# mkln/spamtree

Hardware: AMD Instinct MI355X
Metric: Gibbs iterations/sec + achieved HBM GB/s, n=1e6 grid, 1/2/4/8 MI355X (higher is better)
Workload: dtype f64

## Files before the change

### profiles/micro/stamps.py

```python
import ctypes as C
import os
import sys

import numpy as np

ROOT = os.path.dirname(os.path.dirname(os.path.dirname(os.path.abspath(__file__))))
sys.path.insert(0, ROOT)
from spamtree_amd import _lib

_lib.LIB_PATH = os.path.join(ROOT, "profiles", "micro", "libspamtree_hip_stamps.so")
from spamtree_amd.model import SpamTreeMV
from spamtree_amd.synthetic import make_workload

NAMES = {0: "topology+coords", 1: "covariance", 2: "private ancestor step", 3: "panel barrier wait", 4: "panel compute (MFMA)",
         5: "DMA wait + pad", 6: "DMA issue", 7: "cholesky", 8: "N = -Ri T + store", 9: "final barrier", 10: "hv", 11: "R / leaf outputs",
         12: "Ri out + e2", 13: "scalars"}

side = int(sys.argv[1]) if len(sys.argv) > 1 else 1000
q = int(sys.argv[2]) if len(sys.argv) > 2 else 1
cell = int(sys.argv[3]) if len(sys.argv) > 3 else 25
missing = tuple(float(x) for x in sys.argv[4].split(",")) if len(sys.argv) > 4 else None
wl = make_workload(side, q=q, cell_size=cell, missing=missing, device=0)
hm = SpamTreeMV(wl["y"], wl["X"], wl["Z"], wl["coords"], wl["mv_id"], wl["blocking"], wl["gix_block"], wl["res_is_ref"],
                wl["parents"], wl["children"], False, wl["block_names"], wl["block_groups"], wl["indexing"],
                np.zeros(wl["n"]), np.zeros(wl["p"]), wl["theta"], 10.0, device=0)
lib = hm.lib
lib.st_debug_stamps.argtypes = [C.POINTER(C.c_ulonglong), C.c_int]
lib.st_debug_stamp_level.argtypes = [C.c_int]
hm.get_loglik_comps_w(0)
nlev = len(np.unique(np.asarray(wl["block_groups"])))
for lev in range(max(0, nlev - 4), nlev):
    lib.st_debug_stamp_level(lev)
    buf = (C.c_ulonglong * 16)()
    lib.st_debug_stamps(buf, 1)
    for _ in range(3):
        hm.get_loglik_comps_w(1)
    lib.st_debug_stamps(buf, 0)
    v = np.array(list(buf), dtype=np.float64)
    tot = v.sum()
    if tot == 0:
        continue
    print(f"level {lev}: total ticks {tot:.3e}")
    for i in np.argsort(-v):
        if v[i] > 0:
            print(f"   {NAMES.get(int(i), str(i)):28s} {100 * v[i] / tot:5.1f} %")
hm.close()
```

### spamtree_amd/csrc/factor_quad.hpp

```cpp
#pragma once

struct Quad {
  int g0, nu;
  int Jc, Pc;
};

struct QuadArgs {
  const Blk *blks;
  const int *anc_idx;
  const Grp *grps;
  const Quad *quads;
  int nquad;
  const double *cx, *cy;
  const int *mv;
  const double *w;
  double *panels;
  double *logdet_c, *loglik_c;
  int *errflag;
  const long long *gdesc;
  int gd_stride;
  int ldS;
  int wave_chol;
  int predict;
  const double *z;
  double *w_out;
  int mode;
  double *vscr;
  int vtiles;
};

enum { QM_FULL = 0, QM_VONLY = 1, QM_TFROMV = 2 };
__host__ __device__ constexpr int quad_vtiles(int nkx) { return 2 + 2 * ((4 * nkx + 31) / 32); }

#define RFL(x) __builtin_amdgcn_readfirstlane(x)

constexpr int QUAD_LEAF_KH = 5;
__host__ __device__ constexpr int quad_lds_stride(int nkx) {
  int s = 4 * nkx + 24 > 186 ? 4 * nkx + 24 : 186;
  while ((s & 1) || ((s >> 1) & 1) == 0) ++s;
  return s;
}

#ifdef ST_DEFS_FACTOR_QUAD
__device__ __forceinline__ void dma_row(const double *src, double *dst, int Kb, int lane, bool two) {
  if (2 * lane < Kb) __builtin_amdgcn_global_load_lds((q_glb_void *)(src + 2 * lane), (q_lds_void *)dst, 16, 0, 0);
  if (two) {
    if (128 + 2 * lane < Kb) __builtin_amdgcn_global_load_lds((q_glb_void *)(src + 128 + 2 * lane), (q_lds_void *)(dst + 128), 16, 0, 0);
  }
}

template <int NU, int NKX, int NKT, bool ISREF, bool WCH = true>
__global__ __launch_bounds__(128 * NU, 2) void k_factor_quad(QuadArgs A, CovPar cp) {
  constexpr int NTQ = 128 * NU, NW = 2 * NU;
  static_assert(NU >= 2, "s_g overlays two rows of s_e2");
  constexpr int PMAX = 4 * NKX, KH = ISREF ? (NKX + 3) / 4 : QUAD_LEAF_KH, NPASS = (NKX + KH - 1) / KH;
  static_assert(NKT * 16 >= PMAX, "T tiles must cover the chain");
  extern __shared__ double lds[];
  __shared__ int s_am[MAXJ], s_ao[MAXJ + 1];
  __shared__ long long s_arow[MAXJ], s_apan[MAXJ];
  __shared__ int s_uM[NU], s_uP[NU], s_ublk0[NU], s_unblk[NU], s_uref[NU], s_uJ[NU], s_pm[NU], s_fail[NU], s_level;
  __shared__ long long s_urow0[NU], s_prow[NU], s_ppan[NU];
  constexpr int NB = ISREF ? 1 : 32, NUL = ISREF ? 1 : NU;
  __shared__ long long s_bpan[NU][NB], s_brow[NU][NB];
  __shared__ int s_bld[NU][NB];
  __shared__ double s_colx[NU][32], s_coly[NU][32], s_colw[NU][32], s_hv[NU][32];
  __shared__ double s_px[NUL][32], s_py[NUL][32], s_pw[NUL][32];
  __shared__ double s_e2[NU][32], s_lg[NU][32];
  __shared__ int s_colmv[NU][32], s_colblk[NUL][32], s_pmv[NUL][32];
  __shared__ int s_nit;
  __shared__ double s_sx[PMAX], s_sy[PMAX], s_wpa[PMAX];
  __shared__ int s_smv[PMAX];
  __shared__ double s_exp2[64];
  __shared__ double s_cvr[QMAX * QMAX], s_cva[QMAX * QMAX], s_cva2[QMAX * QMAX], s_cvp[QMAX];
  __shared__ int s_rlen[PMAX];
  __shared__ long long s_rsrc[PMAX];
  double (*s_g)[32] = s_e2;
  double (*s_gp)[32] = s_hv;

  auto body = [&](auto qmc) __attribute__((always_inline)) {
  constexpr int QM = decltype(qmc)::value;
  const int tid = threadIdx.x, lane = tid & 63, l15 = lane & 15, l4 = lane >> 4, ttid = tid & 127;
  const int wid = RFL(tid >> 6), u = wid >> 1, jt = (wid & 1) ^ ((wid >> 2) & 1);
  constexpr int ldS = quad_lds_stride(NKX);
  double *arena = lds;
  double *zrow = arena + (size_t)NU * 16 * ldS;
  double *xch = zrow + ldS;

  STAMP_DECL
  int qidx = blockIdx.x;
  {
    const int per = A.nquad >> 3;
    if (qidx < per * 8) qidx = (qidx & 7) * per + (qidx >> 3);
  }
  const Quad Q = A.quads[qidx];
  const int Jc = Q.Jc, Pc = Q.Pc, nu = Q.nu;

  long long *gdl = (long long *)arena;
  const int gds = A.gd_stride;
  for (int e = tid; e < nu * gds; e += NTQ) {
    const int uu = e / gds, i = e - uu * gds;
    gdl[e] = A.gdesc[(size_t)(Q.g0 + uu) * gds + i];
  }
  for (int k = tid; k < ldS; k += NTQ) zrow[k] = 0.0;
  if (tid < 64) s_exp2[tid] = EXP2_64[tid];
  if (cp.q > 1 && tid >= 64 && tid < 64 + QMAX * QMAX) {
    const int e = tid - 64;
    s_cvr[e] = cp.rate[e]; s_cva[e] = cp.amp[e]; s_cva2[e] = cp.amp2[e];
    if (e < QMAX) s_cvp[e] = cp.phi[e];
  }
  __syncthreads();
  if (tid < NU) {
    int M = 0, P = 0, blk0 = 0, nblk = 0, isref = 0, J = 0, pm = 0;
    long long row0 = 0, prow = 0, ppan = 0;
    if (tid < nu) {
      const long long *g = gdl + (size_t)tid * gds;
      row0 = g[0];
      M = (int)(g[2] & 0xffffffffLL); P = (int)(g[2] >> 32);
      J = (int)(g[3] & 0xffffffffLL); nblk = (int)(g[3] >> 32);
      isref = (int)(g[4] & 0xffffffffLL);
      blk0 = (int)(g[6] & 0xffffffffLL);
      if (tid == 0) s_level = (int)(g[4] >> 32);
      if (J > Jc) {
        const long long *a = g + 8 + 4 * Jc;
        pm = (int)(a[0] & 0xffffffffLL); prow = a[1]; ppan = a[2];
      }
    }
    s_uM[tid] = M; s_uP[tid] = P; s_ublk0[tid] = blk0; s_unblk[tid] = nblk; s_uref[tid] = isref; s_uJ[tid] = J;
    s_pm[tid] = pm; s_urow0[tid] = row0; s_prow[tid] = prow; s_ppan[tid] = ppan; s_fail[tid] = 0;
  }
  if (tid >= 64 && tid < 64 + Jc) {
    const int t = tid - 64;
    const long long *a = gdl + 8 + 4 * t;
    s_am[t] = (int)(a[0] & 0xffffffffLL); s_ao[t] = (int)(a[0] >> 32); s_arow[t] = a[1]; s_apan[t] = a[2];
  }
  if (tid == 32) {
    s_ao[Jc] = Pc;
    s_nit = (Pc + 31) >> 5;
  }
  for (int e = tid; e < NU * NB; e += NTQ) {
    const int uu = e / NB, b = e - uu * NB;
    if (uu < nu) {
      const long long *g = gdl + (size_t)uu * gds;
      const int J = (int)(g[3] & 0xffffffffLL), nblk = (int)(g[3] >> 32);
      if (b < nblk) {
        const long long *q = g + 8 + 4 * J + 3 * b;
        s_bpan[uu][b] = q[0]; s_brow[uu][b] = q[1]; s_bld[uu][b] = (int)q[2];
      }
    }
  }
  __syncthreads();
  const int Mu = RFL(s_uM[u]), Pu = RFL(s_uP[u]), pmu = RFL(s_pm[u]);
  constexpr bool isref = ISREF;
  const bool wact = jt * 16 < Mu;
  const bool two = Mu > 16;
  int Mmax = 0, pmmax = 0;
#pragma unroll
  for (int i = 0; i < NU; ++i) { Mmax = max(Mmax, s_uM[i]); pmmax = max(pmmax, s_pm[i]); }
  Mmax = RFL(Mmax); pmmax = RFL(pmmax);
  constexpr bool anyref = ISREF;

  for (int k = tid; k < Pc; k += NTQ) {
    int t = 0;
#pragma unroll
    for (int j = 1; j < 8; ++j) t += (j < Jc && k >= s_ao[j]) ? 1 : 0;
    for (int j = 8; j < Jc; ++j) t += (k >= s_ao[j]) ? 1 : 0;
    const long long r = s_arow[t] + (k - s_ao[t]);
    s_sx[k] = A.cx[r]; s_sy[k] = A.cy[r]; s_smv[k] = A.mv[r]; s_wpa[k] = A.w[r];
    const int len = s_ao[t + 1];
    s_rlen[k] = len; s_rsrc[k] = s_apan[t] + (long long)(k - s_ao[t]) * len;
  }
  for (int e = tid; e < NU * 32; e += NTQ) {
    const int uu = e >> 5, i = e & 31;
    double x = 0.0, y = 0.0, ww = 0.0; int v = 0;
    if constexpr (!ISREF) {
      if (i < s_pm[uu]) { const long long r = s_prow[uu] + i; x = A.cx[r]; y = A.cy[r]; ww = A.w[r]; v = A.mv[r]; }
      s_px[uu][i] = x; s_py[uu][i] = y; s_pw[uu][i] = ww; s_pmv[uu][i] = v;
      x = 0.0; y = 0.0; ww = 0.0; v = 0;
    }
    int bi = 0;
    if (i < s_uM[uu]) {
      const long long r = s_urow0[uu] + i;
      x = A.cx[r]; y = A.cy[r]; ww = A.w[r]; v = A.mv[r];
      if constexpr (!ISREF) { while (bi + 1 < s_unblk[uu] && r >= s_brow[uu][bi + 1]) ++bi; }
    }
    s_colx[uu][i] = x; s_coly[uu][i] = y; s_colw[uu][i] = ww; s_colmv[uu][i] = v;
    if constexpr (!ISREF) s_colblk[uu][i] = bi;
  }
  __syncthreads();

  STAMP(0);
  const int p_sr0 = pmu > 16 ? (pmu + 1) >> 1 : pmu;
  const int p_Kb = Pc + pmu;
  constexpr int RP = 32 / NW;
  const int nit = RFL(s_nit);
  int rlen_cur[RP], rlen_nx[RP];
#pragma unroll
  for (int rr = 0; rr < RP; ++rr) { rlen_cur[rr] = 0; rlen_nx[rr] = 0; }
  auto issue = [&](int i, double *buf) {
    const int c0 = 32 * (nit - 1 - i), sr = min(32, Pc - c0);
    int lv[RP];
    long long sv[RP];
#pragma unroll
    for (int rr = 0; rr < RP; ++rr) {
// ... 63 lines not shown
            double v = s_cva[ij] * cov_exp_tab(-s_cvr[ij] * hd, s_exp2);
            v = fma(s_cva2[ij], cov_exp_tab(-s_cvp[av] * hd, s_exp2), v);
            kb[i * 64] = (cok && k < Pu) ? v : 0.0;
          }
        }
#pragma unroll
        for (int i = 0; i < KH; ++i)
          if (st0 + i < NKX) kx[st0 + i] = kb[i * 64];
      } else {
#pragma unroll
        for (int i = 0; i < KH; ++i)
          if (st0 + i < NKX) kx[st0 + i] = 0.0;
      }
    }
  }
  STAMP(1);
  d4 tacc[NKT];
#pragma unroll
  for (int n = 0; n < NKT; ++n) tacc[n] = (d4){0.0, 0.0, 0.0, 0.0};
  d4 rown = (d4){0.0, 0.0, 0.0, 0.0}, rcross = rown;
  double dacc = 0.0;
  double hacc = 0.0;
  const size_t vq0 = ((size_t)qidx * A.vtiles * NW + wid) * 256;
  auto vstore = [&](int t, const d4 &p) __attribute__((always_inline)) {
    double *d = A.vscr + (vq0 + (size_t)t * (NW * 256)) + lane;
    __builtin_nontemporal_store(p[0], d); __builtin_nontemporal_store(p[1], d + 64);
    __builtin_nontemporal_store(p[2], d + 128); __builtin_nontemporal_store(p[3], d + 192);
  };
  auto vload = [&](int t) __attribute__((always_inline)) {
    const double *d = A.vscr + (vq0 + (size_t)t * (NW * 256)) + lane;
// ... 98 lines not shown
          double gv = 0.0;
          if (row < sr) gv = grow(buf + (size_t)row * ldS, p_Kb, Pc, s_pw[u], lane & 7, std::integral_constant<int, 8>());
          if ((lane & 7) == 0) s_gp[u][r0 + row] = gv;
        }
        lds_barrier();
        if (sp == 1 && pf) issue(0, arena + (size_t)48 * ldS);
        if (sr > 0) {
          tile(buf, (sr + 3) >> 2, min(p_Kb, Pc + r0 + sr), 0, sr, &s_gp[u][r0], kget(16 + 4 * sp), sp);
        }
        lds_barrier();
      }
    }
  }

  STAMP(2);
  {
    if constexpr (!ISREF) { if (nit > 0 && !pf) issue(0, arena); }
    int cur = pf ? 1 : 0;
    if (QM == QM_TFROMV && wact && nit > 0) { kset(0, vload(2)); if (Pc - 32 * (nit - 1) > 16) kset(4, vload(3)); }
    for (int i = 0; i < nit; ++i) {
      const int c0 = 32 * (nit - 1 - i), sr = min(32, Pc - c0);
      const int kb_v = s_rlen[c0 + sr - 1], kba_v = s_rlen[c0 + min(sr, 16) - 1];
      const int Kb = RFL(kb_v), KbA0 = RFL(kba_v);
      double *buf = arena + (size_t)((pf && i == 0) ? 48 : cur * 32) * ldS;
#pragma unroll
      for (int rr = 0; rr < RP; ++rr) rlen_cur[rr] = rlen_nx[rr];
      asm volatile("s_waitcnt vmcnt(0)" ::: "memory");
#pragma unroll
      for (int rr = 0; rr < RP; ++rr) {
        const int row = wid + NW * rr;
// ... 15 lines not shown
        if (lane % NS == 0) s_g[cur][row] = gv;
      }
      STAMP(5);
      lds_barrier();
      STAMP(3);
      if (i + 1 < nit) issue(i + 1, arena + (size_t)(cur ^ 1) * 32 * ldS);
      if (QM == QM_TFROMV && wact && i + 1 < nit) { kset(8, vload(2 * i + 4)); if (Pc - 32 * (nit - 2 - i) > 16) kset(12, vload(2 * i + 5)); }
      STAMP(6);
      compute(buf, sr, min(Kb, c0 + 32), min(KbA0, c0 + 16), ISREF ? nullptr : s_g[cur], kget(0), kget(4), 2 + 2 * i);
      if (QM == QM_TFROMV) { kset(0, kget(8)); kset(4, kget(12)); }
      STAMP(4);
      cur ^= 1;
    }
  }
  lds_barrier();

  double h0 = 0.0, h1 = 0.0, h2 = 0.0, h3 = 0.0;
  if (QM == QM_FULL && (ISREF || A.predict)) {
#pragma unroll
    for (int n = 0; n < NKT; ++n) {
      const int k = n * 16 + l15;
      double wv = k < Pc ? s_wpa[k] : 0.0;
      if constexpr (!ISREF) { if (k >= Pc && k < Pu) wv = s_pw[u][k - Pc]; }
      h0 += tacc[n][0] * wv; h1 += tacc[n][1] * wv; h2 += tacc[n][2] * wv; h3 += tacc[n][3] * wv;
    }
#pragma unroll
    for (int o = 1; o < 16; o <<= 1) {
      h0 += __shfl_xor(h0, o, 64); h1 += __shfl_xor(h1, o, 64); h2 += __shfl_xor(h2, o, 64); h3 += __shfl_xor(h3, o, 64);
    }
    if (l15 == 0) {
// ... 299 lines not shown
```

### spamtree_amd/csrc/spamtree_hip.hip

```cpp

#include <unordered_map>

#include "tree_layout.hpp"
#include "misc_kernels.hpp"
#include "predict_points.hpp"
#include "predict_joint.hpp"
#include "simulate_kernels.hpp"

static thread_local std::string g_create_error;
struct st_handle_s;
static void points_free(st_handle_s *h);

template <typename T>
struct DevBuf {
  T *p = nullptr;
  size_t n = 0;
  DevBuf() = default;
  DevBuf(const DevBuf &) = delete;
  DevBuf &operator=(const DevBuf &) = delete;
  DevBuf(DevBuf &&o) noexcept : p(o.p), n(o.n) { o.p = nullptr; o.n = 0; }
  DevBuf &operator=(DevBuf &&o) noexcept { if (this != &o) { free(); p = o.p; n = o.n; o.p = nullptr; o.n = 0; } return *this; }
  ~DevBuf() { free(); }
  hipError_t alloc(size_t count) {
    n = count;
// ... 30 lines not shown
  "k_factor_quad<4, 50, 13, true, true>", "k_factor_quad<4, 50, 13, true, false>", "k_factor_quad<4, 50, 13, false, true>",
  "k_factor_mfma", "k_factor_lchain<96>", "k_factor_lchain<136>", "k_factor_ref_finish", "k_lchain_scalars", "k_factor_wide<WG_JT>",
  "k_factor_bigmfma<3, 5, 34>", "k_factor_bigmfma<4, 5, 34>", "k_factor_bigmfma<5, 3, 24>",
  "k_gram", "k_gram_direct", "k_gram_big",
  "k_sample_mfma", "k_sample_leaf_seg<4>", "k_sample_leaf_seg<6>", "k_sample_leaf", "k_sample_wave", "k_sample_lean<true>",
  "k_sample_lean<false>", "k_sample<true, false>", "k_sample_leaf_wide", "k_sample<true, true>", "k_sample<false>",
};

struct st_handle_s : TreeLayout {
  std::string err;
  int device = 0;
  hipStream_t stream = nullptr;
  int quirks = 1;
  long long n_obs = 0;
  DevBuf<Grp> d_grps;
  DevBuf<Quad> d_quads;
  DevBuf<WideGrp> d_wgrps;
  DevBuf<LcSlab> d_lcslabs;
  DevBuf<long long> d_rfvoff, d_gdesc;
  DevBuf<double> d_vscr;
  DevBuf<double> d_lcrow;
  DevBuf<double> d_s0;
  DevBuf<long long> d_s0off;
  bool c_pending = false;
  int c_rc = 0; double c_ll = 0.0;
  DevBuf<int> d_ownobs, d_owngrp, d_ownslow;
  DevBuf<unsigned char> d_rowmask, d_blkmask;
  DevBuf<double> d_comm;
  DevBuf<double> d_gather;
  DevBuf<int> d_gidx;
  DevBuf<double> d_gerr;
// ... 244 lines not shown
  CCHK(h->d_mv.upload(mv)); CCHK(h->d_obs.upload(obs)); CCHK(h->d_partner.upload(partner));
  CCHK(h->d_dev2model.upload(h->dev2model));
  return ST_OK;
}

static int create_layout_buffers(st_handle_s *h) {
  {
    std::vector<Blk> db = h->blks;
    if (h->limited) for (Blk &B : db) B.acc_len = 0;
    CCHK(h->d_blks.upload(db));
    if (h->limited) CCHK(upload_or_dummy(h->d_twin, h->twin_list));
  }
  CCHK(upload_or_dummy(h->d_anc, h->anc_idx)); CCHK(upload_or_dummy(h->d_dch, h->dch_idx));
  CCHK(h->d_lvl.upload(h->lvl_list));
  CCHK(upload_or_dummy(h->d_grps, h->grps)); CCHK(h->d_gdesc.upload(h->gdesc));
  CCHK(upload_or_dummy(h->d_quads, h->quads)); CCHK(upload_or_dummy(h->d_wgrps, h->wgrps));
  if (!h->lcslabs.empty()) { CCHK(h->d_lcslabs.upload(h->lcslabs)); CCHK(h->d_lcrow.alloc((size_t)2 * h->n_all)); }
  if (!h->rfvoff.empty()) { CCHK(h->d_rfvoff.upload(h->rfvoff)); CCHK(h->d_vscr.alloc(h->vscr_need + (size_t)2 * RF_BUFD)); }
  CCHK(h->d_s0off.upload(h->s0off));
  CCHK(h->d_s0.alloc(std::max(h->s0_total, (size_t)1)));
  CCHK(upload_or_dummy(h->d_pred, h->pred_list));
  CCHK(h->d_allobs.upload(h->all_obs_list));
  CCHK(upload_or_dummy(h->d_ownobs, h->own_obs_list));
  CCHK(upload_or_dummy(h->d_owngrp, h->own_grp_list)); CCHK(upload_or_dummy(h->d_ownslow, h->own_obs_slow));
  CCHK(h->d_rowmask.upload(h->rowmask)); CCHK(h->d_blkmask.upload(h->blkmask));
  CCHK(h->d_comm.alloc((size_t)2 * h->n_blocks + 64));
  CCHK(h->d_gidx.upload(h->gidx));
  CCHK(h->d_gather.alloc(h->gidx.size()));
  CCHK(h->d_gerr.alloc(64));
  CCHK(upload_or_dummy(h->d_toplist, h->top_list));
  CCHK(h->d_err2.alloc(2));
// ... 162 lines not shown
  if (h->top_pending) { HCHK(h, hipSetDevice(h->device)); HCHK(h, hipStreamWaitEvent(h->stream, h->ev_top, 0)); }
  return ST_OK;
}
static int complete_leaf(st_handle h, int slot) {
  const int phys = h->slot_map[slot];
  if (!h->leaf_pending[phys]) return ST_OK;
  HCHK(h, hipSetDevice(h->device));
  const CovPar &cp = h->leaf_cp[phys];
  ProfScope phase(h, 0, -2, 0);
  for (int g = 0; g < h->n_actual_groups; ++g) {
    const LevelInfo &L = h->levels[g];
    if (L.vl_off < 0) continue;
    QuadArgs F;
    std::memset(&F, 0, sizeof(F));
    F.blks = h->d_blks.p; F.anc_idx = h->d_anc.p; F.grps = h->d_grps.p + L.grp_first;
    F.quads = h->d_quads.p + L.quad_first + L.qown_lo; F.nquad = L.qown_n;
    F.cx = h->d_cx.p; F.cy = h->d_cy.p; F.mv = h->d_mv.p; F.w = h->d_w.p; F.panels = h->d_panels[phys].p;
    F.errflag = h->d_err.p; F.ldS = L.q_ldS;
    F.gdesc = h->d_gdesc.p + (size_t)L.grp_first * h->gd_stride; F.gd_stride = h->gd_stride;
    F.wave_chol = L.maxM <= 27 ? 1 : 0;
    F.mode = QM_TFROMV; F.vscr = h->d_vleaf.p + L.vl_off; F.vtiles = quad_vtiles(L.q_nkx);
    ProfScope ps(h, 0, g, 0);
#define QT(NU_, NKX_, NKT_) hipLaunchKernelGGL((k_factor_quad<NU_, NKX_, NKT_, false, true>), dim3(L.qown_n), dim3(128 * NU_), L.lds_quad, h->stream, F, cp)
    if (L.q_nkx == 32) QT(4, 32, 8); else if (L.q_nkx == 38) QT(4, 38, 10); else if (L.q_nkx == 44) QT(4, 44, 11); else QT(4, 50, 13);
#undef QT
    HCHK(h, hipGetLastError());
  }
  h->leaf_pending[phys] = false;
  return ST_OK;
}
extern "C" int st_swap(st_handle h) {
  if (!h) return ST_ERR_USAGE;
  if (h->top_pending) {
    h->err = "st_swap between st_factor_begin and the st_factor / st_factor_local that picks its result up";
// ... 116 lines not shown
  for (int g = g_lo; g < g_hi; ++g) {
    const LevelInfo &L = h->levels[g];
    if ((L.fast ? L.gown_n : L.own_n) == 0) continue;
    FactorArgs A;
    std::memset(&A, 0, sizeof(A));
    A.blks = h->d_blks.p; A.anc_idx = h->d_anc.p; A.list = h->d_lvl.p + L.first + L.own_lo; A.nlist = L.own_n;
    A.cx = h->d_cx.p; A.cy = h->d_cy.p; A.mv = h->d_mv.p; A.w_in = h->d_w.p; A.w_out = nullptr; A.z = nullptr;
    A.panels = h->d_panels[phys].p; A.logdet_c = h->d_logdet[phys].p; A.loglik_c = h->d_loglik[phys].p;
    A.errflag = errflag; A.maxP = L.maxP; A.maxM = L.maxM; A.maxMa = L.maxMa; A.SR = L.big_factor ? 4 : 8;
    {
      ProfScope ps(h, 0, g, 1, st);
      if (L.fast && h->sw.factor_gen == 3 && L.q_nkx > 0) {
        QuadArgs F;
        std::memset(&F, 0, sizeof(F));
        F.blks = h->d_blks.p; F.anc_idx = h->d_anc.p; F.grps = h->d_grps.p + L.grp_first;
        F.quads = h->d_quads.p + L.quad_first + L.qown_lo; F.nquad = L.qown_n;
        F.cx = h->d_cx.p; F.cy = h->d_cy.p; F.mv = h->d_mv.p; F.w = h->d_w.p; F.panels = h->d_panels[phys].p;
        F.logdet_c = h->d_logdet[phys].p; F.loglik_c = h->d_loglik[phys].p; F.errflag = errflag; F.ldS = L.q_ldS;
        F.gdesc = h->d_gdesc.p + (size_t)L.grp_first * h->gd_stride; F.gd_stride = h->gd_stride;
        F.wave_chol = L.maxM <= 27 ? 1 : 0;
#define QLAUNCH(NU_, NKX_, NKT_, R_)     \
  do {                                                                                                                         \
    if (L.isref && F.wave_chol) { route(g, R_); hipLaunchKernelGGL((k_factor_quad<NU_, NKX_, NKT_, true, true>), dim3(L.qown_n), dim3(128 * NU_), L.lds_quad, st, F, cp); } \
    else if (L.isref) { route(g, R_ + 1); hipLaunchKernelGGL((k_factor_quad<NU_, NKX_, NKT_, true, false>), dim3(L.qown_n), dim3(128 * NU_), L.lds_quad, st, F, cp); } \
    else {                                                                                                                     \
      if (vonly && L.vl_off >= 0) { F.mode = QM_VONLY; F.vscr = h->d_vleaf.p + L.vl_off; F.vtiles = quad_vtiles(NKX_); *deferred = true; } \
      route(g, R_ + 2); hipLaunchKernelGGL((k_factor_quad<NU_, NKX_, NKT_, false, true>), dim3(L.qown_n), dim3(128 * NU_), L.lds_quad, st, F, cp); } \
  } while (0)
        if (L.q_nkx == 32) QLAUNCH(4, 32, 8, R_QUAD32_REF_WCH); else if (L.q_nkx == 38) QLAUNCH(4, 38, 10, R_QUAD38_REF_WCH);
        else if (L.q_nkx == 44) QLAUNCH(4, 44, 11, R_QUAD44_REF_WCH); else QLAUNCH(4, 50, 13, R_QUAD50_REF_WCH);
#undef QLAUNCH
      } else if (L.fast) {
        FastArgs F;
        std::memset(&F, 0, sizeof(F));
// ... 655 lines not shown
  (void)theta_changed;
  if (!h) return ST_ERR_USAGE;
  if (h->pred_list.empty()) return ST_OK;
  invalidate_stats(h);
  if (!h->z_valid) { h->err = "st_predict needs the normals of a preceding st_sample_w (spamtree_model.cpp:1325)"; return ST_ERR_USAGE; }
  if (h->theta[0].empty()) { h->err = "st_predict before st_factor(slot 0)"; return ST_ERR_USAGE; }
  HCHK(h, hipSetDevice(h->device));
  CovPar cp;
  int rc = make_covpar(h, h->theta[0].data(), (int)h->theta[0].size(), &cp);
  if (rc) return rc;
  const LevelInfo &L = h->pred_info;
  if (h->pred_nkx > 0 && h->pred_quad_count > 0) {
    QuadArgs F;
    std::memset(&F, 0, sizeof(F));
    F.blks = h->d_blks.p; F.anc_idx = h->d_anc.p; F.grps = h->d_grps.p + h->pred_grp_first;
    F.quads = h->d_quads.p + h->pred_quad_first; F.nquad = h->pred_quad_count;
    F.cx = h->d_cx.p; F.cy = h->d_cy.p; F.mv = h->d_mv.p; F.w = h->d_w.p; F.panels = h->d_panels[h->slot_map[0]].p;
    F.logdet_c = nullptr; F.loglik_c = nullptr; F.errflag = h->d_err.p; F.ldS = quad_lds_stride(h->pred_nkx);
    F.gdesc = h->d_gdesc.p + (size_t)h->pred_grp_first * h->gd_stride; F.gd_stride = h->gd_stride;
    F.wave_chol = 1; F.predict = 1; F.z = h->d_z.p; F.w_out = h->d_w.p;
    {
      ProfScope ps(h, 6);
      const dim3 grid(h->pred_quad_count), blk(128 * 4);
      if (h->pred_nkx == 32) { h->route_p = R_QUAD32_LEAF; hipLaunchKernelGGL((k_factor_quad<4, 32, 8, false, true>), grid, blk, h->pred_lds, h->stream, F, cp); }
      else if (h->pred_nkx == 38) { h->route_p = R_QUAD38_LEAF; hipLaunchKernelGGL((k_factor_quad<4, 38, 10, false, true>), grid, blk, h->pred_lds, h->stream, F, cp); }
      else if (h->pred_nkx == 44) { h->route_p = R_QUAD44_LEAF; hipLaunchKernelGGL((k_factor_quad<4, 44, 11, false, true>), grid, blk, h->pred_lds, h->stream, F, cp); }
      else { h->route_p = R_QUAD50_LEAF; hipLaunchKernelGGL((k_factor_quad<4, 50, 13, false, true>), grid, blk, h->pred_lds, h->stream, F, cp); }
    }
    HCHK(h, hipGetLastError());
    HCHK(h, hipStreamSynchronize(h->stream));
    return ST_OK;
  }
  FactorArgs A;
  std::memset(&A, 0, sizeof(A));
// ... 991 lines not shown
```

### spamtree_amd/csrc/tree_layout.cpp

```cpp
#include "tree_layout.hpp"

Switches read_switches() {
  auto level = [](const char *name) {
    const char *e = getenv(name);
    return (e && e[0] == '0') ? 0 : ((e && e[0] == '2') ? 2 : 1);
  };
  Switches s;
  s.wide = level("SPAMTREE_WIDE"); s.split_gram = level("SPAMTREE_SPLIT_GRAM"); s.sample_wave = level("SPAMTREE_SAMPLE_WAVE");
  s.lchain = level("SPAMTREE_LCHAIN"); s.lchain_ref = level("SPAMTREE_LCHAIN_REF"); s.gram_big = level("SPAMTREE_GRAM_BIG");
  s.gram_direct = level("SPAMTREE_GRAM_DIRECT"); s.sample_lean = level("SPAMTREE_SAMPLE_LEAN"); s.sample_lat = level("SPAMTREE_SAMPLE_LAT");
  s.leaf_seg = level("SPAMTREE_LEAF_SEG"); s.leaf_wide = level("SPAMTREE_LEAF_WIDE"); s.async_top = level("SPAMTREE_ASYNC_TOP");
  const char *e;
  if ((e = getenv("SPAMTREE_LCHAIN_REF_MIN"))) s.lchain_ref_min = atoi(e);
  if ((e = getenv("SPAMTREE_FACTOR_KERNEL")) && e[0] == '1') s.factor_gen = 1;
  if ((e = getenv("SPAMTREE_QUAD_UNITS"))) s.quad_units = atoi(e);
  if ((e = getenv("SPAMTREE_QUAD_MIN"))) s.quad_min = std::max(atoi(e), 0);
  return s;
}

static int refuse(std::string &msg, int code, const std::string &text) { msg = text; return code; }

static size_t lds_factor_bytes(int maxP, int maxM, int maxMa, int SR, bool big) {
  size_t dbl = (size_t)3 * (maxP + maxM) + 3 * (size_t)maxM + (size_t)SR * maxP;
  size_t bytes = dbl * 8 + (size_t)((maxP + maxM + 1) & ~1) * 4;
// ... 691 lines not shown
    if (L.lchain_ref) {
      L.lds_ref_finish = rf_lds_bytes(L.maxM);
      if (L.lds_ref_finish > t.lds_limit) { L.lchain = 0; L.lchain_ref = false; }
    }
  }
  for (auto &L : t.levels)
    if (L.q_nkx && L.lds_quad + dl.quad_static > DeviceLimits::CU_LDS) L.q_nkx = 0;
  if (t.pred_nkx && t.pred_lds + dl.quad_static > DeviceLimits::CU_LDS) t.pred_nkx = 0;
  for (auto &L : t.levels) {
    L.vl_off = -1;
    if (!t.defer_leaf || t.world > 1 || t.limited || t.sw.factor_gen != 3 || !L.fast || L.isref || L.q_nkx == 0 || L.qown_n == 0) continue;
    L.vl_off = (long long)t.vleaf_total;
    t.vleaf_total += (size_t)L.qown_n * quad_vtiles(L.q_nkx) * (2 * t.quad_nu) * 256;
  }
}
static void choose_top_levels(TreeLayout &t) {
  const int n_actual = t.n_actual_groups;
  t.g_top = 0;
  bool all_fast = !t.limited && !t.force_generic;
  for (int g = 0; g < n_actual; ++g) all_fast = all_fast && t.levels[g].fast;
  if (all_fast) {
    while (t.g_top < n_actual && !(t.sw.factor_gen == 3 && t.levels[t.g_top].q_nkx > 0)) ++t.g_top;
    if (t.g_top >= n_actual) t.g_top = 0;
  }
  for (int b : t.own_obs_list) if (t.blks[b].level < t.g_top) t.top_list.push_back(b);
  t.n_toplist = (int)t.top_list.size();
}

int layout_levels(const st_problem *pb, const Switches &sw, const DeviceLimits &dl, TreeLayout &t, std::string &msg) {
  t.sw = sw;
// ... 12 lines not shown
    level_wide_groups(t, L);
    level_lchain_slabs(t, L);
    level_quads(t, L, g);
  }
  mark_owned(t);
  if (int rc = build_prediction(t, msg)) return rc;
  for (long long r = 0; r < t.n_all; ++r)
    if (pb->mv_id[r] < 1 || pb->mv_id[r] > pb->q) return refuse(msg, ST_ERR_USAGE, "mv_id out of range");
  std::vector<long long> blk2grp((size_t)t.n_blocks, -1);
  for (size_t g = 0; g < t.grps.size(); ++g)
    for (int b = 0; b < t.grps[g].nblk; ++b) blk2grp[t.grps[g].blk0 + b] = (long long)g;
  if (int rc = pack_group_descriptors(t, blk2grp, msg)) return rc;
  choose_gram_direct(t, blk2grp);
  size_buffers(t);
  demote_by_static_lds(t, dl);
  choose_top_levels(t);
  return ST_OK;
}
```

### spamtree_amd/csrc/tree_layout.hpp

```cpp
#pragma once
#include "st_device.hpp"
#include "factor_generic.hpp"
#include "factor_mfma.hpp"
#include "chol_blocked.hpp"
#include "factor_quad.hpp"
#include "factor_big.hpp"
#include "factor_wide.hpp"
#include "factor_lchain.hpp"
#include "sample_kernels.hpp"

struct LevelInfo {
  int first = 0, count = 0;
  int isref = 1;
  int maxP = 0, maxM = 0, maxMa = 0, maxLd = 0;
  bool big_factor = false, big_sample = false, sample_sq = false;
  size_t lds_factor = 0, lds_sample = 0, lds_loglik = 0;
  double alg_bytes_A = 0, alg_bytes_B = 0, alg_bytes_C = 0, alg_bytes_msg = 0;
  double flops_A = 0, flops_B = 0, flops_C = 0;
  bool fast = false;
  int grp_first = 0, grp_count = 0, Pm4 = 0, ldKV = 2, ldS = 2, SRm = 1, stage_dbl = 0;
  size_t lds_fast = 0;
  int ldN = 2, Mr4 = 4, Mrows = 1, av_dbl = 224, maxJ = 0;
  size_t lds_sfast = 0, lds_slean = 0;
  bool bigmfma = false;
  int wide_first = 0, wide_count = 0, wide_maxN = 0;
  size_t lds_wide = 0;
  int bm_ldS = 0;
  size_t lds_bigmfma = 0;
  int lchain = 0;
  bool lchain_ref = false;
  size_t lds_ref_finish = 0;
  int rf_first = 0;
  int lc_first = 0, lc_count = 0;
  int quad_first = 0, quad_count = 0, qown_lo = 0, qown_n = 0, q_ldS = 0, q_nkx = 0;
  long long vl_off = -1;
  size_t lds_quad = 0;
  int own_lo = 0, own_n = 0, gown_lo = 0, gown_n = 0;
};

struct Switches {
  int wide = 1, split_gram = 1, sample_wave = 1;
  bool lchain = true, lchain_ref = true, gram_big = true, gram_direct = true, sample_lean = true, sample_lat = true,
       leaf_seg = true, leaf_wide = true, async_top = true;
  int lchain_ref_min = 1;
  int factor_gen = 3;
  int quad_units = 0;
  int quad_min = -1;
};
Switches read_switches();
// ... 13 lines not shown
  int q = 1, p = 1, d = 2, n_groups = 0, n_actual_groups = 0;
  int force_generic = 0;
  bool limited = false;
  bool defer_leaf = false;
  Switches sw;
  size_t lds_limit = 65536;
  int sm_count = 256;
  int quad_nu = 4;

  std::vector<long long> dev2model, model2dev;
  std::vector<int> blk_model2dev;
  std::vector<Blk> blks;
  std::vector<int> anc_idx, dch_idx, lvl_list, pred_list, all_obs_list;
  std::vector<Grp> grps;
  std::vector<Quad> quads;
  std::vector<WideGrp> wgrps;
  std::vector<LcSlab> lcslabs;
  std::vector<long long> rfvoff;
  size_t vscr_need = 0;
  std::vector<long long> gdesc;
  int gd_stride = 8;
  std::vector<long long> s0off;
  size_t s0_total = 0;
  int rank = 0, world = 1, cut = 0;
  std::vector<int> blk_owner;
  std::vector<int> own_obs_list;
  std::vector<int> own_grp_list, own_obs_slow;
  std::vector<unsigned char> rowmask, blkmask;
  std::vector<int> gidx;
  int gather_cnt = 1;
// ... 22 lines not shown
```

Baseline: 243.9.

## Precompute per-quad records on host and DMA them into LDS in one shot

Builds a fixed-layout per-quad record on the host at layout time. It holds unit metadata, block panel descriptors, coordinates, multivariate ids, and row indices in place of w values. The kernel loads the whole record into LDS with direct global-to-LDS loads instead of decoding gdesc and gathering coordinates through several dependent passes and barriers. Only w values are fetched per call, through the parked row indices. This removes serialized setup latency and gathers in the factor prologue, at the cost of extra device memory for the records and a fixed record size tied to the NKX variants. It also adds register-pinning asm for the ISREF non-WCH variant and extends the profiling script.

```diff
diff --git a/profiles/micro/stamps.py b/profiles/micro/stamps.py
--- a/profiles/micro/stamps.py
+++ b/profiles/micro/stamps.py
@@ -8,7 +8,7 @@
 sys.path.insert(0, ROOT)
 from spamtree_amd import _lib
 
-_lib.LIB_PATH = os.path.join(ROOT, "profiles", "micro", "libspamtree_hip_stamps.so")
+_lib.LIB_PATH = os.environ.get("SPAMTREE_STAMPS_LIB") or os.path.join(ROOT, "profiles", "micro", "libspamtree_hip_stamps.so")
 from spamtree_amd.model import SpamTreeMV
 from spamtree_amd.synthetic import make_workload
 
@@ -19,7 +19,8 @@
 side = int(sys.argv[1]) if len(sys.argv) > 1 else 1000
 q = int(sys.argv[2]) if len(sys.argv) > 2 else 1
 cell = int(sys.argv[3]) if len(sys.argv) > 3 else 25
-missing = tuple(float(x) for x in sys.argv[4].split(",")) if len(sys.argv) > 4 else None
+missing = tuple(float(x) for x in sys.argv[4].split(",")) if len(sys.argv) > 4 and sys.argv[4] != "-" else None
+vonly = len(sys.argv) > 5 and sys.argv[5] == "vonly"
 wl = make_workload(side, q=q, cell_size=cell, missing=missing, device=0)
 hm = SpamTreeMV(wl["y"], wl["X"], wl["Z"], wl["coords"], wl["mv_id"], wl["blocking"], wl["gix_block"], wl["res_is_ref"],
                 wl["parents"], wl["children"], False, wl["block_names"], wl["block_groups"], wl["indexing"],
@@ -28,19 +29,32 @@
 lib.st_debug_stamps.argtypes = [C.POINTER(C.c_ulonglong), C.c_int]
 lib.st_debug_stamp_level.argtypes = [C.c_int]
 hm.get_loglik_comps_w(0)
+hm.get_loglik_comps_w(1)
+theta1 = np.ascontiguousarray(hm.theta[1], dtype=np.float64)
+
+
+def factor():
+    if not vonly:
+        hm.get_loglik_comps_w(1)
+        return
+    ll = C.c_double()
+    assert lib.st_factor_enqueue(hm.h, 1, theta1.ctypes.data_as(C.POINTER(C.c_double)), theta1.size) == 0
+    assert lib.st_factor_finish(hm.h, C.byref(ll)) == 0
+
+
 nlev = len(np.unique(np.asarray(wl["block_groups"])))
 for lev in range(max(0, nlev - 4), nlev):
     lib.st_debug_stamp_level(lev)
     buf = (C.c_ulonglong * 16)()
     lib.st_debug_stamps(buf, 1)
     for _ in range(3):
-        hm.get_loglik_comps_w(1)
+        factor()
     lib.st_debug_stamps(buf, 0)
     v = np.array(list(buf), dtype=np.float64)
     tot = v.sum()
     if tot == 0:
         continue
-    print(f"level {lev}: total ticks {tot:.3e}")
+    print(f"level {lev}{' (proposal)' if vonly else ''}: total ticks {tot:.3e}")
     for i in np.argsort(-v):
         if v[i] > 0:
             print(f"   {NAMES.get(int(i), str(i)):28s} {100 * v[i] / tot:5.1f} %")
diff --git a/spamtree_amd/csrc/factor_quad.hpp b/spamtree_amd/csrc/factor_quad.hpp
--- a/spamtree_amd/csrc/factor_quad.hpp
+++ b/spamtree_amd/csrc/factor_quad.hpp
@@ -9,7 +9,8 @@
   const Blk *blks;
   const int *anc_idx;
   const Grp *grps;
-  const Quad *quads;
+  const long long *qrec;
+  int qrec_stride;
   int nquad;
   const double *cx, *cy;
   const int *mv;
@@ -17,8 +18,6 @@
   double *panels;
   double *logdet_c, *loglik_c;
   int *errflag;
-  const long long *gdesc;
-  int gd_stride;
   int ldS;
   int wave_chol;
   int predict;
@@ -32,6 +31,35 @@
 enum { QM_FULL = 0, QM_VONLY = 1, QM_TFROMV = 2 };
 __host__ __device__ constexpr int quad_vtiles(int nkx) { return 2 + 2 * ((4 * nkx + 31) / 32); }
 
+template <int NU, int PMAX, bool ISREF>
+struct alignas(16) QuadRec {
+  static constexpr int NB = ISREF ? 1 : 32, NUL = ISREF ? 1 : NU, NLD = ISREF ? 2 : 32, NLI = ISREF ? 4 : 32;
+  int g0, nu, Jc, Pc;
+  int level, nit, pad[2];
+  int uM[NU], uP[NU], ublk0[NU], unblk[NU], uref[NU], uJ[NU], pm[NU], fail[NU];
+  long long urow0[NU], prow[NU], ppan[NU];
+  long long bpan[NU][NB], brow[NU][NB];
+  int bld[NU][NB];
+  double colx[NU][32], coly[NU][32], colw[NU][32];
+  int colmv[NU][32], colblk[NUL][NLI];
+  double px[NUL][NLD], py[NUL][NLD], pw[NUL][NLD];
+  int pmv[NUL][NLI];
+  double sx[PMAX], sy[PMAX], wpa[PMAX];
+  int smv[PMAX];
+  int rlen[PMAX];
+  long long rsrc[PMAX];
+};
+static_assert(sizeof(QuadRec<4, 128, true>) % 16 == 0 && sizeof(QuadRec<4, 152, false>) % 16 == 0 && sizeof(QuadRec<4, 176, true>) % 16 == 0 &&
+              sizeof(QuadRec<4, 200, false>) % 16 == 0, "a record is a whole number of 16-byte DMA pieces");
+inline int quad_rec_words(int nkx, bool isref) {
+  switch (nkx) {
+    case 32: return (int)((isref ? sizeof(QuadRec<4, 128, true>) : sizeof(QuadRec<4, 128, false>)) / 8);
+    case 38: return (int)((isref ? sizeof(QuadRec<4, 152, true>) : sizeof(QuadRec<4, 152, false>)) / 8);
+    case 44: return (int)((isref ? sizeof(QuadRec<4, 176, true>) : sizeof(QuadRec<4, 176, false>)) / 8);
+    default: return (int)((isref ? sizeof(QuadRec<4, 200, true>) : sizeof(QuadRec<4, 200, false>)) / 8);
+  }
+}
+
 #define RFL(x) __builtin_amdgcn_readfirstlane(x)
 
 constexpr int QUAD_LEAF_KH = 5;
@@ -56,24 +84,22 @@
   constexpr int PMAX = 4 * NKX, KH = ISREF ? (NKX + 3) / 4 : QUAD_LEAF_KH, NPASS = (NKX + KH - 1) / KH;
   static_assert(NKT * 16 >= PMAX, "T tiles must cover the chain");
   extern __shared__ double lds[];
-  __shared__ int s_am[MAXJ], s_ao[MAXJ + 1];
-  __shared__ long long s_arow[MAXJ], s_apan[MAXJ];
-  __shared__ int s_uM[NU], s_uP[NU], s_ublk0[NU], s_unblk[NU], s_uref[NU], s_uJ[NU], s_pm[NU], s_fail[NU], s_level;
-  __shared__ long long s_urow0[NU], s_prow[NU], s_ppan[NU];
   constexpr int NB = ISREF ? 1 : 32, NUL = ISREF ? 1 : NU;
-  __shared__ long long s_bpan[NU][NB], s_brow[NU][NB];
-  __shared__ int s_bld[NU][NB];
-  __shared__ double s_colx[NU][32], s_coly[NU][32], s_colw[NU][32], s_hv[NU][32];
-  __shared__ double s_px[NUL][32], s_py[NUL][32], s_pw[NUL][32];
+  typedef QuadRec<NU, PMAX, ISREF> Rec;
+  static_assert(PMAX <= NTQ / 2 && NU * 32 * 2 <= NTQ / 2, "one parked w per thread: chain | columns | private rows");
+  __shared__ Rec s_q;
+  auto &s_uM = s_q.uM; auto &s_uP = s_q.uP; auto &s_ublk0 = s_q.ublk0; auto &s_unblk = s_q.unblk; auto &s_uJ = s_q.uJ;
+  auto &s_pm = s_q.pm; auto &s_fail = s_q.fail; auto &s_level = s_q.level; auto &s_nit = s_q.nit;
+  auto &s_urow0 = s_q.urow0; auto &s_ppan = s_q.ppan;
+  auto &s_bpan = s_q.bpan; auto &s_brow = s_q.brow; auto &s_bld = s_q.bld;
+  auto &s_colx = s_q.colx; auto &s_coly = s_q.coly; auto &s_colw = s_q.colw; auto &s_colmv = s_q.colmv; auto &s_colblk = s_q.colblk;
+  auto &s_px = s_q.px; auto &s_py = s_q.py; auto &s_pw = s_q.pw; auto &s_pmv = s_q.pmv;
+  auto &s_sx = s_q.sx; auto &s_sy = s_q.sy; auto &s_wpa = s_q.wpa; auto &s_smv = s_q.smv;
+  auto &s_rlen = s_q.rlen; auto &s_rsrc = s_q.rsrc;
+  __shared__ double s_hv[NU][32];
   __shared__ double s_e2[NU][32], s_lg[NU][32];
-  __shared__ int s_colmv[NU][32], s_colblk[NUL][32], s_pmv[NUL][32];
-  __shared__ int s_nit;
-  __shared__ double s_sx[PMAX], s_sy[PMAX], s_wpa[PMAX];
-  __shared__ int s_smv[PMAX];
   __shared__ double s_exp2[64];
   __shared__ double s_cvr[QMAX * QMAX], s_cva[QMAX * QMAX], s_cva2[QMAX * QMAX], s_cvp[QMAX];
-  __shared__ int s_rlen[PMAX];
-  __shared__ long long s_rsrc[PMAX];
   double (*s_g)[32] = s_e2;
   double (*s_gp)[32] = s_hv;
 
@@ -92,14 +118,15 @@
     const int per = A.nquad >> 3;
     if (qidx < per * 8) qidx = (qidx & 7) * per + (qidx >> 3);
   }
-  const Quad Q = A.quads[qidx];
-  const int Jc = Q.Jc, Pc = Q.Pc, nu = Q.nu;
-
-  long long *gdl = (long long *)arena;
-  const int gds = A.gd_stride;
-  for (int e = tid; e < nu * gds; e += NTQ) {
-    const int uu = e / gds, i = e - uu * gds;
-    gdl[e] = A.gdesc[(size_t)(Q.g0 + uu) * gds + i];
+  {
+    constexpr int NPIECE = (int)(sizeof(Rec) / 16);
+    const char *rec = (const char *)(A.qrec + (size_t)qidx * A.qrec_stride);
+    char *img = (char *)&s_q;
+#pragma unroll
+    for (int p0 = 0; p0 < NPIECE; p0 += 64 * NW) {
+      const int pw0 = p0 + 64 * wid;
+      if (pw0 + lane < NPIECE) __builtin_amdgcn_global_load_lds((q_glb_void *)(rec + (size_t)(pw0 + lane) * 16), (q_lds_void *)(img + (size_t)pw0 * 16), 16, 0, 0);
+    }
   }
   for (int k = tid; k < ldS; k += NTQ) zrow[k] = 0.0;
   if (tid < 64) s_exp2[tid] = EXP2_64[tid];
@@ -108,47 +135,9 @@
     s_cvr[e] = cp.rate[e]; s_cva[e] = cp.amp[e]; s_cva2[e] = cp.amp2[e];
     if (e < QMAX) s_cvp[e] = cp.phi[e];
   }
+  asm volatile("s_waitcnt vmcnt(0)" ::: "memory");
   __syncthreads();
-  if (tid < NU) {
-    int M = 0, P = 0, blk0 = 0, nblk = 0, isref = 0, J = 0, pm = 0;
-    long long row0 = 0, prow = 0, ppan = 0;
-    if (tid < nu) {
-      const long long *g = gdl + (size_t)tid * gds;
-      row0 = g[0];
-      M = (int)(g[2] & 0xffffffffLL); P = (int)(g[2] >> 32);
-      J = (int)(g[3] & 0xffffffffLL); nblk = (int)(g[3] >> 32);
-      isref = (int)(g[4] & 0xffffffffLL);
-      blk0 = (int)(g[6] & 0xffffffffLL);
-      if (tid == 0) s_level = (int)(g[4] >> 32);
-      if (J > Jc) {
-        const long long *a = g + 8 + 4 * Jc;
-        pm = (int)(a[0] & 0xffffffffLL); prow = a[1]; ppan = a[2];
-      }
-    }
-    s_uM[tid] = M; s_uP[tid] = P; s_ublk0[tid] = blk0; s_unblk[tid] = nblk; s_uref[tid] = isref; s_uJ[tid] = J;
-    s_pm[tid] = pm; s_urow0[tid] = row0; s_prow[tid] = prow; s_ppan[tid] = ppan; s_fail[tid] = 0;
-  }
-  if (tid >= 64 && tid < 64 + Jc) {
-    const int t = tid - 64;
-    const long long *a = gdl + 8 + 4 * t;
-    s_am[t] = (int)(a[0] & 0xffffffffLL); s_ao[t] = (int)(a[0] >> 32); s_arow[t] = a[1]; s_apan[t] = a[2];
-  }
-  if (tid == 32) {
-    s_ao[Jc] = Pc;
-    s_nit = (Pc + 31) >> 5;
-  }
-  for (int e = tid; e < NU * NB; e += NTQ) {
-    const int uu = e / NB, b = e - uu * NB;
-    if (uu < nu) {
-      const long long *g = gdl + (size_t)uu * gds;
-      const int J = (int)(g[3] & 0xffffffffLL), nblk = (int)(g[3] >> 32);
-      if (b < nblk) {
-        const long long *q = g + 8 + 4 * J + 3 * b;
-        s_bpan[uu][b] = q[0]; s_brow[uu][b] = q[1]; s_bld[uu][b] = (int)q[2];
-      }
-    }
-  }
-  __syncthreads();
+  const int Pc = RFL(s_q.Pc);
   const int Mu = RFL(s_uM[u]), Pu = RFL(s_uP[u]), pmu = RFL(s_pm[u]);
   constexpr bool isref = ISREF;
   const bool wact = jt * 16 < Mu;
@@ -159,34 +148,21 @@
   Mmax = RFL(Mmax); pmmax = RFL(pmmax);
   constexpr bool anyref = ISREF;
 
-  for (int k = tid; k < Pc; k += NTQ) {
-    int t = 0;
-#pragma unroll
-    for (int j = 1; j < 8; ++j) t += (j < Jc && k >= s_ao[j]) ? 1 : 0;
-    for (int j = 8; j < Jc; ++j) t += (k >= s_ao[j]) ? 1 : 0;
-    const long long r = s_arow[t] + (k - s_ao[t]);
-    s_sx[k] = A.cx[r]; s_sy[k] = A.cy[r]; s_smv[k] = A.mv[r]; s_wpa[k] = A.w[r];
-    const int len = s_ao[t + 1];
-    s_rlen[k] = len; s_rsrc[k] = s_apan[t] + (long long)(k - s_ao[t]) * len;
-  }
-  for (int e = tid; e < NU * 32; e += NTQ) {
-    const int uu = e >> 5, i = e & 31;
-    double x = 0.0, y = 0.0, ww = 0.0; int v = 0;
-    if constexpr (!ISREF) {
-      if (i < s_pm[uu]) { const long long r = s_prow[uu] + i; x = A.cx[r]; y = A.cy[r]; ww = A.w[r]; v = A.mv[r]; }
-      s_px[uu][i] = x; s_py[uu][i] = y; s_pw[uu][i] = ww; s_pmv[uu][i] = v;
-      x = 0.0; y = 0.0; ww = 0.0; v = 0;
-    }
-    int bi = 0;
-    if (i < s_uM[uu]) {
-      const long long r = s_urow0[uu] + i;
-      x = A.cx[r]; y = A.cy[r]; ww = A.w[r]; v = A.mv[r];
-      if constexpr (!ISREF) { while (bi + 1 < s_unblk[uu] && r >= s_brow[uu][bi + 1]) ++bi; }
-    }
-    s_colx[uu][i] = x; s_coly[uu][i] = y; s_colw[uu][i] = ww; s_colmv[uu][i] = v;
-    if constexpr (!ISREF) s_colblk[uu][i] = bi;
-  }
-  __syncthreads();
+  double wpark = 0.0;
+  constexpr int o_wpa = (int)(offsetof(Rec, wpa) / 8), o_colw = (int)(offsetof(Rec, colw) / 8), o_pw = (int)(offsetof(Rec, pw) / 8);
+  auto wslot = [&]() __attribute__((always_inline)) {
+    if (tid < Pc) return o_wpa + tid;
+    if (tid >= NTQ / 2 && tid < NTQ / 2 + 32 * NU) return o_colw + (tid - NTQ / 2);
+    if (!ISREF && tid >= NTQ / 2 + 32 * NU) return o_pw + (tid - (NTQ / 2 + 32 * NU));
+    return -1;
+  };
+  if (QM != QM_TFROMV) {
+    const int ws = wslot();
+    if (ws >= 0) {
+      const long long r = __double_as_longlong(((const double *)&s_q)[ws]);
+      if (r >= 0) wpark = A.w[r];
+    }
+  }
 
   STAMP(0);
   const int p_sr0 = pmu > 16 ? (pmu + 1) >> 1 : pmu;
@@ -280,6 +256,11 @@
       }
     }
   }
+  if (QM != QM_TFROMV) {
+    const int ws = wslot();
+    if (ws >= 0) ((double *)&s_q)[ws] = wpark;
+    if constexpr (!ISREF) lds_barrier();
+  }
   STAMP(1);
   d4 tacc[NKT];
 #pragma unroll
@@ -408,6 +389,10 @@
   }
 
   STAMP(2);
+  if constexpr (ISREF && !WCH) {
+#pragma unroll
+    for (int n = 0; n < NKT; ++n) asm volatile("" : "+v"(tacc[n]));
+  }
   {
     if constexpr (!ISREF) { if (nit > 0 && !pf) issue(0, arena); }
     int cur = pf ? 1 : 0;
@@ -453,6 +438,10 @@
     }
   }
   lds_barrier();
+  if constexpr (ISREF && !WCH) {
+#pragma unroll
+    for (int n = 0; n < NKT; ++n) asm volatile("" : "+v"(tacc[n]));
+  }
 
   double h0 = 0.0, h1 = 0.0, h2 = 0.0, h3 = 0.0;
   if (QM == QM_FULL && (ISREF || A.predict)) {
diff --git a/spamtree_amd/csrc/spamtree_hip.hip b/spamtree_amd/csrc/spamtree_hip.hip
--- a/spamtree_amd/csrc/spamtree_hip.hip
+++ b/spamtree_amd/csrc/spamtree_hip.hip
@@ -68,7 +68,7 @@
   int quirks = 1;
   long long n_obs = 0;
   DevBuf<Grp> d_grps;
-  DevBuf<Quad> d_quads;
+  DevBuf<long long> d_qrec;
   DevBuf<WideGrp> d_wgrps;
   DevBuf<LcSlab> d_lcslabs;
   DevBuf<long long> d_rfvoff, d_gdesc;
@@ -343,7 +343,8 @@
   CCHK(upload_or_dummy(h->d_anc, h->anc_idx)); CCHK(upload_or_dummy(h->d_dch, h->dch_idx));
   CCHK(h->d_lvl.upload(h->lvl_list));
   CCHK(upload_or_dummy(h->d_grps, h->grps)); CCHK(h->d_gdesc.upload(h->gdesc));
-  CCHK(upload_or_dummy(h->d_quads, h->quads)); CCHK(upload_or_dummy(h->d_wgrps, h->wgrps));
+  CCHK(upload_or_dummy(h->d_qrec, h->qrec)); std::vector<long long>().swap(h->qrec);
+  CCHK(upload_or_dummy(h->d_wgrps, h->wgrps));
   if (!h->lcslabs.empty()) { CCHK(h->d_lcslabs.upload(h->lcslabs)); CCHK(h->d_lcrow.alloc((size_t)2 * h->n_all)); }
   if (!h->rfvoff.empty()) { CCHK(h->d_rfvoff.upload(h->rfvoff)); CCHK(h->d_vscr.alloc(h->vscr_need + (size_t)2 * RF_BUFD)); }
   CCHK(h->d_s0off.upload(h->s0off));
@@ -536,10 +537,9 @@
     QuadArgs F;
     std::memset(&F, 0, sizeof(F));
     F.blks = h->d_blks.p; F.anc_idx = h->d_anc.p; F.grps = h->d_grps.p + L.grp_first;
-    F.quads = h->d_quads.p + L.quad_first + L.qown_lo; F.nquad = L.qown_n;
+    F.qrec = L.qr_off >= 0 ? h->d_qrec.p + L.qr_off : nullptr; F.qrec_stride = L.qr_words; F.nquad = L.qown_n;
     F.cx = h->d_cx.p; F.cy = h->d_cy.p; F.mv = h->d_mv.p; F.w = h->d_w.p; F.panels = h->d_panels[phys].p;
     F.errflag = h->d_err.p; F.ldS = L.q_ldS;
-    F.gdesc = h->d_gdesc.p + (size_t)L.grp_first * h->gd_stride; F.gd_stride = h->gd_stride;
     F.wave_chol = L.maxM <= 27 ? 1 : 0;
     F.mode = QM_TFROMV; F.vscr = h->d_vleaf.p + L.vl_off; F.vtiles = quad_vtiles(L.q_nkx);
     ProfScope ps(h, 0, g, 0);
@@ -686,10 +686,9 @@
         QuadArgs F;
         std::memset(&F, 0, sizeof(F));
         F.blks = h->d_blks.p; F.anc_idx = h->d_anc.p; F.grps = h->d_grps.p + L.grp_first;
-        F.quads = h->d_quads.p + L.quad_first + L.qown_lo; F.nquad = L.qown_n;
+        F.qrec = L.qr_off >= 0 ? h->d_qrec.p + L.qr_off : nullptr; F.qrec_stride = L.qr_words; F.nquad = L.qown_n;
         F.cx = h->d_cx.p; F.cy = h->d_cy.p; F.mv = h->d_mv.p; F.w = h->d_w.p; F.panels = h->d_panels[phys].p;
         F.logdet_c = h->d_logdet[phys].p; F.loglik_c = h->d_loglik[phys].p; F.errflag = errflag; F.ldS = L.q_ldS;
-        F.gdesc = h->d_gdesc.p + (size_t)L.grp_first * h->gd_stride; F.gd_stride = h->gd_stride;
         F.wave_chol = L.maxM <= 27 ? 1 : 0;
 #define QLAUNCH(NU_, NKX_, NKT_, R_)     \
   do {                                                                                                                         \
@@ -1375,10 +1374,9 @@
     QuadArgs F;
     std::memset(&F, 0, sizeof(F));
     F.blks = h->d_blks.p; F.anc_idx = h->d_anc.p; F.grps = h->d_grps.p + h->pred_grp_first;
-    F.quads = h->d_quads.p + h->pred_quad_first; F.nquad = h->pred_quad_count;
+    F.qrec = h->d_qrec.p + h->pred_qr_off; F.qrec_stride = h->pred_qr_words; F.nquad = h->pred_quad_count;
     F.cx = h->d_cx.p; F.cy = h->d_cy.p; F.mv = h->d_mv.p; F.w = h->d_w.p; F.panels = h->d_panels[h->slot_map[0]].p;
     F.logdet_c = nullptr; F.loglik_c = nullptr; F.errflag = h->d_err.p; F.ldS = quad_lds_stride(h->pred_nkx);
-    F.gdesc = h->d_gdesc.p + (size_t)h->pred_grp_first * h->gd_stride; F.gd_stride = h->gd_stride;
     F.wave_chol = 1; F.predict = 1; F.z = h->d_z.p; F.w_out = h->d_w.p;
     {
       ProfScope ps(h, 6);
diff --git a/spamtree_amd/csrc/tree_layout.cpp b/spamtree_amd/csrc/tree_layout.cpp
--- a/spamtree_amd/csrc/tree_layout.cpp
+++ b/spamtree_amd/csrc/tree_layout.cpp
@@ -729,6 +729,82 @@
     t.vleaf_total += (size_t)L.qown_n * quad_vtiles(L.q_nkx) * (2 * t.quad_nu) * 256;
   }
 }
+template <int PMAX, bool ISREF>
+static void fill_quad_record(const st_problem *pb, const TreeLayout &t, int grp_first, const Quad &Qd, long long *out) {
+  typedef QuadRec<4, PMAX, ISREF> Rec;
+  Rec R;
+  std::memset(&R, 0, sizeof(R));
+  const long long n = t.n_all;
+  auto put = [&](long long r, double &x, double &y, int &mv, double &wslot) {
+    const long long m = t.dev2model[r];
+    x = pb->coords[m]; y = pb->coords[n + m]; mv = (int)(pb->mv_id[m] - 1);
+    std::memcpy(&wslot, &r, sizeof(double));
+  };
+  const long long none = -1;
+  for (int i = 0; i < 4 * 32; ++i) std::memcpy(&R.colw[0][0] + i, &none, sizeof(double));
+  for (int i = 0; i < Rec::NUL * Rec::NLD; ++i) std::memcpy(&R.pw[0][0] + i, &none, sizeof(double));
+  for (int k = 0; k < PMAX; ++k) std::memcpy(&R.wpa[k], &none, sizeof(double));
+  R.g0 = Qd.g0; R.nu = Qd.nu; R.Jc = Qd.Jc; R.Pc = Qd.Pc;
+  R.nit = (Qd.Pc + 31) >> 5;
+  const Blk &U0 = t.blks[t.grps[grp_first + Qd.g0].blk0];
+  R.level = U0.level;
+  int k = 0;
+  for (int a = 0; a < Qd.Jc; ++a) {
+    const Blk &Ba = t.blks[t.anc_idx[U0.anc_ptr + a]];
+    const int len = k + Ba.m;
+    for (int i = 0; i < Ba.m && k < PMAX; ++i, ++k) {
+      put(Ba.row0 + i, R.sx[k], R.sy[k], R.smv[k], R.wpa[k]);
+      R.rlen[k] = len; R.rsrc[k] = Ba.chain_off + (long long)i * len;
+    }
+  }
+  for (int u = 0; u < Qd.nu; ++u) {
+    const Grp &G = t.grps[grp_first + Qd.g0 + u];
+    const Blk &B0 = t.blks[G.blk0];
+    R.uM[u] = G.M; R.uP[u] = G.P; R.ublk0[u] = G.blk0; R.unblk[u] = G.nblk; R.uref[u] = B0.isref; R.uJ[u] = B0.nanc; R.urow0[u] = G.row0;
+    if (B0.nanc > Qd.Jc) {
+      const Blk &Bp = t.blks[t.anc_idx[B0.anc_ptr + Qd.Jc]];
+      R.pm[u] = Bp.m; R.prow[u] = Bp.row0; R.ppan[u] = Bp.chain_off;
+      if constexpr (!ISREF) for (int i = 0; i < Bp.m && i < 32; ++i) put(Bp.row0 + i, R.px[u][i], R.py[u][i], R.pmv[u][i], R.pw[u][i]);
+    }
+    for (int b = 0; b < G.nblk && b < Rec::NB; ++b) {
+      const Blk &Bb = t.blks[G.blk0 + b];
+      R.bpan[u][b] = Bb.panel_off; R.brow[u][b] = Bb.row0; R.bld[u][b] = Bb.ld;
+    }
+    int bi = 0;
+    for (int i = 0; i < G.M && i < 32; ++i) {
+      put(G.row0 + i, R.colx[u][i], R.coly[u][i], R.colmv[u][i], R.colw[u][i]);
+      if constexpr (!ISREF) {
+        while (bi + 1 < G.nblk && G.row0 + i >= t.blks[G.blk0 + bi + 1].row0) ++bi;
+        R.colblk[u][i] = bi;
+      }
+    }
+  }
+  std::memcpy(out, &R, sizeof(R));
+}
+static long long append_quad_records(const st_problem *pb, TreeLayout &t, int grp_first, int qfirst, int count, int nkx, bool isref, int &words) {
+  words = quad_rec_words(nkx, isref);
+  const long long off = (long long)t.qrec.size();
+  t.qrec.resize(t.qrec.size() + (size_t)count * words);
+  for (int k = 0; k < count; ++k) {
+    long long *out = t.qrec.data() + off + (size_t)k * words;
+    const Quad &Qd = t.quads[qfirst + k];
+#define QR(P_) (isref ? fill_quad_record<P_, true>(pb, t, grp_first, Qd, out) : fill_quad_record<P_, false>(pb, t, grp_first, Qd, out))
+    if (nkx == 32) QR(128); else if (nkx == 38) QR(152); else if (nkx == 44) QR(176); else QR(200);
+#undef QR
+  }
+  return off;
+}
+static void build_quad_records(const st_problem *pb, TreeLayout &t) {
+  t.qrec.clear(); t.pred_qr_off = -1; t.pred_qr_words = 0;
+  for (auto &L : t.levels) {
+    L.qr_off = -1; L.qr_words = 0;
+    if (t.sw.factor_gen != 3 || !L.fast || L.q_nkx == 0 || L.qown_n == 0) continue;
+    L.qr_off = append_quad_records(pb, t, L.grp_first, L.quad_first + L.qown_lo, L.qown_n, L.q_nkx, L.isref != 0, L.qr_words);
+  }
+  if (t.pred_nkx && t.pred_quad_count > 0)
+    t.pred_qr_off = append_quad_records(pb, t, t.pred_grp_first, t.pred_quad_first, t.pred_quad_count, t.pred_nkx, false, t.pred_qr_words);
+  t.qrec_bytes = t.qrec.size() * sizeof(long long);
+}
 static void choose_top_levels(TreeLayout &t) {
   const int n_actual = t.n_actual_groups;
   t.g_top = 0;
@@ -771,6 +847,7 @@
   choose_gram_direct(t, blk2grp);
   size_buffers(t);
   demote_by_static_lds(t, dl);
+  build_quad_records(pb, t);
   choose_top_levels(t);
   return ST_OK;
 }
diff --git a/spamtree_amd/csrc/tree_layout.hpp b/spamtree_amd/csrc/tree_layout.hpp
--- a/spamtree_amd/csrc/tree_layout.hpp
+++ b/spamtree_amd/csrc/tree_layout.hpp
@@ -33,6 +33,8 @@
   int rf_first = 0;
   int lc_first = 0, lc_count = 0;
   int quad_first = 0, quad_count = 0, qown_lo = 0, qown_n = 0, q_ldS = 0, q_nkx = 0;
+  long long qr_off = -1;
+  int qr_words = 0;
   long long vl_off = -1;
   size_t lds_quad = 0;
   int own_lo = 0, own_n = 0, gown_lo = 0, gown_n = 0;
@@ -76,6 +78,10 @@
   std::vector<int> anc_idx, dch_idx, lvl_list, pred_list, all_obs_list;
   std::vector<Grp> grps;
   std::vector<Quad> quads;
+  std::vector<long long> qrec;
+  size_t qrec_bytes = 0;
+  long long pred_qr_off = -1;
+  int pred_qr_words = 0;
   std::vector<WideGrp> wgrps;
   std::vector<LcSlab> lcslabs;
   std::vector<long long> rfvoff;
```

Result: faster. 249.0 (median of 6 runs) (+2.1%).
